# ska-sa/dc_sand

Measured on AMD Instinct MI355X. Metric: Gcoeff/s (complex weights) 64ant x 1024beam x 32768chan per GPU, higher is better.
Workload: dtype f32

## Files before the change

### dc_sand_amd/csrc/bf_capi_stream.hip

```cpp

#include <cstring>
#include <new>

#include "../../include/dcs_stream_staging.h"
#include "bf_stream_ext.h"
#include "bf_host.h"

using namespace bf_host;

constexpr int kTableRing = 4;
struct dcs_bf_stream {
    bf_stream_ext_head ext;
    dcs_bf_context *ctx;
    hipStream_t stream;
    hipGraph_t graph;
    hipGraphExec_t exec;
    hipGraphNode_t node;
    bf_kernel_launch launch;
    bool has_terms;
    hipGraphNode_t terms_node;
    bf_terms_args terms_args;
    const void *terms_func;
    dim3 terms_grid, terms_block;
    dcs_delay_vals *h_table[kTableRing];
    hipEvent_t table_copied[kTableRing];
    bool table_pending[kTableRing];
    int table_next;
    hipGraph_t ggraph;
    hipGraphExec_t gexec;
    hipGraphNode_t gnode_gather, gnode_terms, gnode_gen;
    bf_gather_launch gather;
    dcs_delay_vals *d_spare;
    hipStream_t stage_stream;
    hipEvent_t staged_ev;
    hipEvent_t released_ev;
    bool released_recorded;
    bool staged;
};

namespace {

void kernel_node_params(const bf_kernel_launch &l, void **params, hipKernelNodeParams *np)
{
    std::memset(np, 0, sizeof(*np));
    np->func = const_cast<void *>(l.func);
    np->gridDim = l.grid;
    np->blockDim = l.block;
    np->sharedMemBytes = l.shared;
    np->kernelParams = params;
    np->extra = nullptr;
}

void terms_node_params(const dcs_bf_stream *s, void **params, hipKernelNodeParams *tp)
{
    std::memset(tp, 0, sizeof(*tp));
    tp->func = const_cast<void *>(s->terms_func);
    tp->gridDim = s->terms_grid;
    tp->blockDim = s->terms_block;
    tp->kernelParams = params;
}

void gather_node_params(dcs_bf_stream *s, void **params, hipKernelNodeParams *gp)
{
    bf_gather_launch &g = s->gather;
    params[0] = &g.local;
    params[1] = &g.global;
    params[2] = &g.n_ant;
    params[3] = &g.nb_local;
    params[4] = &g.nb_total;
    params[5] = &g.beam_offset;
    std::memset(gp, 0, sizeof(*gp));
    gp->func = const_cast<void *>(g.func);
    gp->gridDim = g.grid;
    gp->blockDim = g.block;
    gp->kernelParams = params;
}

int build_stream_graph(dcs_bf_stream *s, bool with_gather, hipGraph_t *graph, hipGraphExec_t *exec, hipGraphNode_t *n_gather,
                       hipGraphNode_t *n_terms, hipGraphNode_t *n_gen)
{
    DCS_TRY(hipGraphCreate(graph, 0));
    hipGraphNode_t prev = nullptr;
    if (with_gather) {
        void *gparams[6];
        hipKernelNodeParams gp;
        gather_node_params(s, gparams, &gp);
        DCS_TRY(hipGraphAddKernelNode(n_gather, *graph, nullptr, 0, &gp));
        prev = *n_gather;
    }
    if (s->has_terms) {
        void *tparams[] = {&s->terms_args};
        hipKernelNodeParams tp;
        terms_node_params(s, tparams, &tp);
        DCS_TRY(hipGraphAddKernelNode(n_terms, *graph, prev ? &prev : nullptr, prev ? 1 : 0, &tp));
        prev = *n_terms;
    }
    void *params[] = {&s->launch.args};
    hipKernelNodeParams np;
    kernel_node_params(s->launch, params, &np);
    DCS_TRY(hipGraphAddKernelNode(n_gen, *graph, prev ? &prev : nullptr, prev ? 1 : 0, &np));
    DCS_TRY(hipGraphInstantiate(exec, *graph, nullptr, nullptr, 0));
    return DCS_OK;
}

int replay(dcs_bf_stream *s, float dt, const dcs_delay_vals *delays, hipGraphExec_t exec, hipGraphNode_t n_gather,
           hipGraphNode_t n_terms, hipGraphNode_t n_gen)
{
    s->launch.args.a.dt0 = dt;
    s->launch.args.a.delays = delays;
    if (n_gather) {
        void *gparams[6];
        hipKernelNodeParams gp;
        gather_node_params(s, gparams, &gp);
        DCS_TRY(hipGraphExecKernelNodeSetParams(exec, n_gather, &gp));
    }
    if (s->has_terms) {
        s->terms_args.dt0 = dt;
        s->terms_args.dt_inline[0] = dt;
        s->terms_args.delays = delays;
        void *tparams[] = {&s->terms_args};
        hipKernelNodeParams tp;
        terms_node_params(s, tparams, &tp);
        DCS_TRY(hipGraphExecKernelNodeSetParams(exec, n_terms, &tp));
    }
    void *params[] = {&s->launch.args};
    hipKernelNodeParams np;
    kernel_node_params(s->launch, params, &np);
    DCS_TRY(hipGraphExecKernelNodeSetParams(exec, n_gen, &np));
    return (int)hipGraphLaunch(exec, s->stream);
}

int ensure_staging(dcs_bf_stream *s)
{
    if (!s->d_spare) DCS_TRY(hipMalloc((void **)&s->d_spare, (size_t)s->ctx->n_pairs * sizeof(dcs_delay_vals)));
    if (!s->stage_stream) {
        int least = 0, greatest = 0;
        DCS_TRY(hipDeviceGetStreamPriorityRange(&least, &greatest));
        DCS_TRY(hipStreamCreateWithPriority(&s->stage_stream, hipStreamNonBlocking, greatest));
    }
    if (!s->staged_ev) DCS_TRY(hipEventCreateWithFlags(&s->staged_ev, hipEventDisableTiming));
    if (!s->released_ev) DCS_TRY(hipEventCreateWithFlags(&s->released_ev, hipEventDisableTiming));
    return DCS_OK;
}

int begin_staging(dcs_bf_stream *s)
{
    const int cap = refuse_if_capturing(s->stream);
    if (cap != DCS_OK) return cap;
    const int st = ensure_staging(s);
    if (st != DCS_OK) return st;
    if (s->released_recorded) DCS_TRY(hipStreamWaitEvent(s->stage_stream, s->released_ev, 0));
    return DCS_OK;
}

int consume_staged(dcs_bf_stream *s, float dt)
{
    dcs_bf_context *c = s->ctx;
    DCS_TRY(hipStreamWaitEvent(s->stream, s->staged_ev, 0));
    DCS_TRY(hipEventRecord(s->released_ev, s->stream));
    s->released_recorded = true;
    const int st = replay(s, dt, s->d_spare, s->exec, nullptr, s->terms_node, s->node);
    if (st != DCS_OK) return st;
    dcs_delay_vals *retired = c->d_table[c->cur];
    c->d_table[c->cur] = s->d_spare;
    s->d_spare = retired;
    s->staged = false;
    return DCS_OK;
}

int stage_table_impl(dcs_bf_stream *s, const dcs_delay_vals *table, int flags)
{
    if (!s || !table) return DCS_ERR_INVALID_ARGUMENT;
    if (flags != 0 && flags != DCS_BF_STAGE_CALLER_PINNED) return DCS_ERR_INVALID_ARGUMENT;
    dcs_bf_context *c = s->ctx;
    DCS_CHECK_DEVICE(c);
    const size_t tb = (size_t)c->n_pairs * sizeof(dcs_delay_vals);
    const int st = begin_staging(s);
    if (st != DCS_OK) return st;
    const void *src = table;
    int r = -1;
    if (flags == 0) {
        r = s->table_next;
        s->table_next = (r + 1) % kTableRing;
        if (s->table_pending[r]) DCS_TRY(hipEventSynchronize(s->table_copied[r]));
        std::memcpy(s->h_table[r], table, tb);
        src = s->h_table[r];
    }
    DCS_TRY(hipMemcpyAsync(s->d_spare, src, tb, hipMemcpyHostToDevice, s->stage_stream));
    if (r >= 0) {
        DCS_TRY(hipEventRecord(s->table_copied[r], s->stage_stream));
        s->table_pending[r] = true;
    }
    DCS_TRY(hipEventRecord(s->staged_ev, s->stage_stream));
    s->staged = true;
    return DCS_OK;
}

int stage_table_from_global_impl(dcs_bf_stream *s, const void *d_global, uint32_t nb_total, uint32_t beam_offset,
                                 void *ready_event)
{
    if (!s || !d_global) return DCS_ERR_INVALID_ARGUMENT;
    dcs_bf_context *c = s->ctx;
    DCS_CHECK_DEVICE(c);
    if ((uint64_t)beam_offset + (uint64_t)c->p.nr_beams > nb_total) return DCS_ERR_OUT_OF_RANGE;
    if ((reinterpret_cast<uintptr_t>(d_global) & 15u) != 0) return DCS_ERR_INVALID_ARGUMENT;
    const int st = begin_staging(s);
    if (st != DCS_OK) return st;
    if (ready_event) DCS_TRY(hipStreamWaitEvent(s->stage_stream, reinterpret_cast<hipEvent_t>(ready_event), 0));
    DCS_TRY(bf_launch_gather_beams(s->d_spare, static_cast<const dcs_delay_vals *>(d_global), (uint32_t)c->p.nr_stations,
                                   (uint32_t)c->p.nr_beams, nb_total, beam_offset, s->stage_stream));
    DCS_TRY(hipEventRecord(s->staged_ev, s->stage_stream));
    s->staged = true;
    return DCS_OK;
}

const bf_stream_ext_ops kStagingOps = {BF_STREAM_EXT_VERSION, stage_table_impl, stage_table_from_global_impl};

}

extern "C" {

int dcs_bf_stream_begin(dcs_bf_context *c, int bitwidth, uint32_t c0, uint32_t nc, void *d_out, size_t out_bytes,
                        void *stream, dcs_bf_stream **out)
{
    if (!c || !out || !d_out) return DCS_ERR_INVALID_ARGUMENT;
    DCS_CHECK_DEVICE(c);
    *out = nullptr;
    if (bitwidth != DCS_BF_B16 && bitwidth != DCS_BF_B32) return DCS_ERR_INVALID_ARGUMENT;
    if (!c->table_set) return DCS_ERR_NOT_READY;
    if ((uint64_t)c0 + nc > (uint64_t)c->p.nr_channels || nc == 0) return DCS_ERR_OUT_OF_RANGE;
    const bool out16 = bitwidth == DCS_BF_B16;
    if (out_bytes < (size_t)nc * c->n_pairs * (out16 ? 4 : 8)) return DCS_ERR_INVALID_ARGUMENT;
    {
        const int cap = refuse_if_capturing(as_stream(stream));
        if (cap != DCS_OK) return cap;
    }

    dcs_bf_stream *s = new (std::nothrow) dcs_bf_stream();
    if (!s) return (int)hipErrorOutOfMemory;
    std::memset(static_cast<void *>(s), 0, sizeof(*s));
    s->ext.ops = &kStagingOps;
    s->ctx = c;
    s->stream = as_stream(stream);
    int st = DCS_OK;
    do {
        s->has_terms = want_terms_table(c, out16, pick_geometry(c, out16, nc, 1), nc, 1);
        if ((st = prepare_tiled(c, out16, nullptr, 0.0f, 1, c0, nc, d_out, &s->launch, nullptr, s->has_terms)) != 0) break;
        if (s->launch.func == nullptr) { st = DCS_ERR_INVALID_ARGUMENT; break; }
        if (s->has_terms) {
            fill_terms_table_args(c, out16, 0.0f, 1, c0, nc, d_out, nullptr, &s->terms_args);
            if ((st = (int)bf_prepare_terms(s->terms_args, &s->terms_func, &s->terms_grid, &s->terms_block)) != 0) break;
            if (s->terms_func == nullptr) { st = DCS_ERR_INVALID_ARGUMENT; break; }
        }
        if ((st = (int)bf_prepare_gather_beams(c->d_table[c->cur ^ 1], c->d_table[c->cur], (uint32_t)c->p.nr_stations,
                                               (uint32_t)c->p.nr_beams, (uint32_t)c->p.nr_beams, 0u, &s->gather)) != 0) break;
        if (s->gather.func == nullptr) { st = DCS_ERR_INVALID_ARGUMENT; break; }
        for (int i = 0; i < kTableRing && st == 0; i++) {
            st = (int)hipHostMalloc((void **)&s->h_table[i], (size_t)c->n_pairs * sizeof(dcs_delay_vals), hipHostMallocDefault);
            if (st == 0) st = (int)hipEventCreateWithFlags(&s->table_copied[i], hipEventDisableTiming);
        }
        if (st != 0) break;
        if ((st = build_stream_graph(s, false, &s->graph, &s->exec, nullptr, &s->terms_node, &s->node)) != 0) break;
        if ((st = build_stream_graph(s, true, &s->ggraph, &s->gexec, &s->gnode_gather, &s->gnode_terms, &s->gnode_gen)) != 0) break;
    } while (0);
    if (st != 0) {
        dcs_bf_stream_end(s);
        return st;
    }
    *out = s;
    return DCS_OK;
}

int dcs_bf_stream_tick_dt(dcs_bf_stream *s, float dt, const dcs_delay_vals *new_table)
{
    if (!s) return DCS_ERR_INVALID_ARGUMENT;
    dcs_bf_context *c = s->ctx;
    DCS_CHECK_DEVICE(c);
    if (s->staged) return new_table ? DCS_ERR_INVALID_ARGUMENT : consume_staged(s, dt);
    if (new_table) {
        const int r = s->table_next;
        s->table_next = (r + 1) % kTableRing;
        if (s->table_pending[r]) DCS_TRY(hipEventSynchronize(s->table_copied[r]));
        std::memcpy(s->h_table[r], new_table, (size_t)c->n_pairs * sizeof(dcs_delay_vals));
        const int nxt = c->cur ^ 1;
        DCS_TRY(hipMemcpyAsync(c->d_table[nxt], s->h_table[r], (size_t)c->n_pairs * sizeof(dcs_delay_vals),
                               hipMemcpyHostToDevice, s->stream));
        DCS_TRY(hipEventRecord(s->table_copied[r], s->stream));
        s->table_pending[r] = true;
        c->cur = nxt;
    }
    return replay(s, dt, c->d_table[c->cur], s->exec, nullptr, s->terms_node, s->node);
}

int dcs_bf_stream_tick(dcs_bf_stream *s, uint64_t t, const dcs_delay_vals *new_table)
{
    if (!s) return DCS_ERR_INVALID_ARGUMENT;
    float dt;
    const int st = dcs_bf_delta_times(&s->ctx->p, t, 1, &dt);
    if (st != DCS_OK) return st;
    return dcs_bf_stream_tick_dt(s, dt, new_table);
}

int dcs_bf_stream_tick_at(dcs_bf_stream *s, const struct timespec *cur, const struct timespec *ref,
                          const dcs_delay_vals *new_table)
{
    if (!s) return DCS_ERR_INVALID_ARGUMENT;
    float dt;
    const int st = dcs_bf_ts_diff(ref, cur, &dt);
    if (st != DCS_OK) return st;
    return dcs_bf_stream_tick_dt(s, dt, new_table);
}

int dcs_bf_stream_tick_dt_from_global(dcs_bf_stream *s, float dt, const void *d_global, uint32_t nb_total, uint32_t beam_offset)
{
    if (!s || !d_global) return DCS_ERR_INVALID_ARGUMENT;
    dcs_bf_context *c = s->ctx;
    DCS_CHECK_DEVICE(c);
    if ((uint64_t)beam_offset + (uint64_t)c->p.nr_beams > nb_total) return DCS_ERR_OUT_OF_RANGE;
    if ((reinterpret_cast<uintptr_t>(d_global) & 15u) != 0) return DCS_ERR_INVALID_ARGUMENT;
    if (s->staged) return DCS_ERR_INVALID_ARGUMENT;
    const int nxt = c->cur ^ 1;
    s->gather.local = c->d_table[nxt];
    s->gather.global = static_cast<const dcs_delay_vals *>(d_global);
    s->gather.nb_total = nb_total;
    s->gather.beam_offset = beam_offset;
    c->cur = nxt;
    return replay(s, dt, c->d_table[c->cur], s->gexec, s->gnode_gather, s->gnode_terms, s->gnode_gen);
}

int dcs_bf_stream_tick_from_global(dcs_bf_stream *s, uint64_t t, const void *d_global, uint32_t nb_total, uint32_t beam_offset)
{
    if (!s) return DCS_ERR_INVALID_ARGUMENT;
    float dt;
    const int st = dcs_bf_delta_times(&s->ctx->p, t, 1, &dt);
    if (st != DCS_OK) return st;
    return dcs_bf_stream_tick_dt_from_global(s, dt, d_global, nb_total, beam_offset);
}

int dcs_bf_stream_tick_at_from_global(dcs_bf_stream *s, const struct timespec *cur, const struct timespec *ref,
                                      const void *d_global, uint32_t nb_total, uint32_t beam_offset)
{
    if (!s) return DCS_ERR_INVALID_ARGUMENT;
    float dt;
    const int st = dcs_bf_ts_diff(ref, cur, &dt);
    if (st != DCS_OK) return st;
    return dcs_bf_stream_tick_dt_from_global(s, dt, d_global, nb_total, beam_offset);
}

int dcs_bf_stream_end(dcs_bf_stream *s)
{
    if (!s) return DCS_OK;
    (void)hipStreamSynchronize(s->stream);
    if (s->stage_stream) {
        (void)hipStreamSynchronize(s->stage_stream);
        (void)hipStreamDestroy(s->stage_stream);
    }
    if (s->staged_ev) (void)hipEventDestroy(s->staged_ev);
    if (s->released_ev) (void)hipEventDestroy(s->released_ev);
    if (s->d_spare) (void)hipFree(s->d_spare);
    if (s->exec) (void)hipGraphExecDestroy(s->exec);
    if (s->graph) (void)hipGraphDestroy(s->graph);
    if (s->gexec) (void)hipGraphExecDestroy(s->gexec);
    if (s->ggraph) (void)hipGraphDestroy(s->ggraph);
    for (int i = 0; i < kTableRing; i++) {
        if (s->table_copied[i]) (void)hipEventDestroy(s->table_copied[i]);
        if (s->h_table[i]) (void)hipHostFree(s->h_table[i]);
    }
    delete s;
    return DCS_OK;
}

}
```

### include/dcs_probes.h

```cpp
#ifndef DCS_PROBES_H
#define DCS_PROBES_H

#include "dcs_beamformer.h"

#ifdef __cplusplus
extern "C" {
#endif
#pragma GCC visibility push(default)

struct dcs_probe_knobs {
    int32_t nomath;
    int32_t pace;
    int32_t fail_at_step;
    int32_t bacc_probe;
    int32_t bacc_rounds;
    int32_t bacc_no_share;
    int32_t bacc_plain;
    int32_t bacc_wg_per_cu;
    int32_t bacc_unstaged;
    int32_t bacc_order;
    int32_t bacc_nbt;
    int32_t bacc_waves;
};
int dcs_probe_set_knobs(dcs_bf_context *ctx, const struct dcs_probe_knobs *k);

int dcs_probe_sincos(int which, const float *d_x, size_t n, float *d_sin, float *d_cos, void *stream);
int dcs_probe_fill(void *d_out, size_t bytes, int nontemporal, void *stream);
int dcs_probe_store_pattern(void *d_out, uint32_t rows, uint32_t cols_kib, uint32_t qb, uint32_t rb, int order,
                            int xcd_remap, int nontemporal, uint32_t block_threads, void *stream);

int dcs_probe_one_store(void *d_out, size_t bytes, int store_mode, int stores_per_thread, uint32_t row_bytes, void *stream);

int dcs_probe_reduce(const void *d_in, size_t bytes, uint64_t *checksum, float *max_modulus_dev, void *stream);

int dcs_probe_mfma(int which, uint32_t blocks, uint32_t iters, float *d_out, void *stream);

uint32_t dcs_probe_xcd_grouped(uint32_t w, uint32_t total, uint32_t group);

int dcs_probe_copy(const void *d_in, void *d_out, size_t bytes, int store_mode, int per_thread, void *stream);

#pragma GCC visibility pop
#ifdef __cplusplus
}
#endif
#endif
```

### probes/dcs_probes.py

```python
from __future__ import annotations

import ctypes
from ctypes import POINTER, byref, c_float, c_int, c_size_t, c_uint32, c_uint64, c_void_p

import numpy as np

from .build import LIB, build

_VP = c_void_p
SIGNATURES = [
    ("dcs_probe_sincos", c_int, [c_int, _VP, c_size_t, _VP, _VP, _VP]),
    ("dcs_probe_fill", c_int, [_VP, c_size_t, c_int, _VP]),
    ("dcs_probe_copy", c_int, [_VP, _VP, c_size_t, c_int, c_int, _VP]),
    ("dcs_probe_one_store", c_int, [_VP, c_size_t, c_int, c_int, c_uint32, _VP]),
    ("dcs_probe_reduce", c_int, [_VP, c_size_t, POINTER(c_uint64), POINTER(c_float), _VP]),
    ("dcs_probe_mfma", c_int, [c_int, c_uint32, c_uint32, _VP, _VP]),
    ("dcs_probe_store_pattern", c_int, [_VP, c_uint32, c_uint32, c_uint32, c_uint32, c_int, c_int, c_int, c_uint32, _VP]),
    ("dcs_probe_set_knobs", c_int, [_VP, _VP]),
    ("dcs_probe_xcd_grouped", c_uint32, [c_uint32, c_uint32, c_uint32]),
]

KNOB_FIELDS = ("nomath", "pace", "fail_at_step", "bacc_probe", "bacc_rounds", "bacc_no_share", "bacc_plain", "bacc_wg_per_cu",
               "bacc_unstaged", "bacc_order", "bacc_nbt", "bacc_waves")

_LIB = None


def lib() -> ctypes.CDLL:
    global _LIB
    if _LIB is None:
        if not LIB.exists():
            build()
        L = ctypes.CDLL(str(LIB))
        for name, restype, argtypes in SIGNATURES:
            fn = getattr(L, name)
            fn.restype = restype
            fn.argtypes = argtypes
        _LIB = L
    return _LIB


def _check(status: int, where: str) -> None:
    if status != 0:
        raise RuntimeError(f"{where}: status {status}")


def _s(stream) -> c_void_p:
    if stream is None:
        return c_void_p(None)
    return c_void_p(int(getattr(stream, "handle", stream)))


def tensor_properties(d_ptr, nbytes: int, stream=None) -> tuple[int, float]:
    ck = c_uint64(0)
    dev = c_float(0.0)
    _check(lib().dcs_probe_reduce(c_void_p(int(d_ptr)), int(nbytes), byref(ck), byref(dev), _s(stream)), "dcs_probe_reduce")
    return int(ck.value), float(dev.value)


def sincos(which: int, d_x, n: int, d_sin, d_cos, stream=None) -> None:
    _check(lib().dcs_probe_sincos(int(which), c_void_p(int(d_x)), int(n), c_void_p(int(d_sin)), c_void_p(int(d_cos)), _s(stream)),
           "dcs_probe_sincos")


def fill(d_out, nbytes: int, nontemporal: int = 1, stream=None) -> None:
    _check(lib().dcs_probe_fill(c_void_p(int(d_out)), int(nbytes), int(nontemporal), _s(stream)), "dcs_probe_fill")


def copy(d_in, d_out, nbytes: int, store_mode: int = 1, per_thread: int = 1, stream=None) -> None:
    _check(lib().dcs_probe_copy(c_void_p(int(d_in)), c_void_p(int(d_out)), int(nbytes), int(store_mode), int(per_thread), _s(stream)),
           "dcs_probe_copy")


def store_pattern(d_out, rows, cols_kib, qb, rb, order=0, xcd_remap=0, store_mode=1, block_threads=256, stream=None) -> None:
    _check(lib().dcs_probe_store_pattern(c_void_p(int(d_out)), rows, cols_kib, qb, rb, order, xcd_remap, store_mode, block_threads,
                                         _s(stream)), "dcs_probe_store_pattern")


def one_store(d_out, nbytes, store_mode, stores_per_thread, row_bytes, stream=None) -> None:
    _check(lib().dcs_probe_one_store(c_void_p(int(d_out)), int(nbytes), int(store_mode), int(stores_per_thread), int(row_bytes),
                                     _s(stream)), "dcs_probe_one_store")


def mfma(which: int, blocks: int, iters: int, d_out, stream=None) -> None:
    _check(lib().dcs_probe_mfma(int(which), int(blocks), int(iters), c_void_p(int(d_out)), _s(stream)), "dcs_probe_mfma")


def set_knobs(gen, **knobs) -> None:
    from dc_sand_amd import _lib as product

    if product.LIB_PATH.resolve() != LIB.resolve():
        raise RuntimeError("set_knobs needs the probes build behind the wrappers: run with DCS_LIB_PATH=probes/libdcs_probes.so")
    unknown = set(knobs) - set(KNOB_FIELDS)
    if unknown:
        raise TypeError(f"unknown knob(s) {sorted(unknown)}")
    if not knobs:
        _check(lib().dcs_probe_set_knobs(c_void_p(gen._h), c_void_p(None)), "dcs_probe_set_knobs")
        return
    k = (ctypes.c_int32 * len(KNOB_FIELDS))(*[int(knobs.get(f, 0)) for f in KNOB_FIELDS])
    _check(lib().dcs_probe_set_knobs(c_void_p(gen._h), ctypes.cast(k, c_void_p)), "dcs_probe_set_knobs")
```

Before: 927.9.

## Route host-table ticks through the staging stream and add stream-join probe knob

When a tick carries a new host delay table, the upload now goes on the high-priority staging stream and joins the compute stream through events, instead of being copied inline on the compute stream. The aim is to let the H2D copy overlap the previous generation kernel rather than serialize ahead of it. A probe knob adds variants that drop the wait, drop or move the release event, or disable the system fence, for measuring the join cost. This adds event record and wait calls per tick, and the no-wait and no-release probe variants give up ordering guarantees.

```diff
diff --git a/dc_sand_amd/csrc/bf_capi_stream.hip b/dc_sand_amd/csrc/bf_capi_stream.hip
--- a/dc_sand_amd/csrc/bf_capi_stream.hip
+++ b/dc_sand_amd/csrc/bf_capi_stream.hip
@@ -130,6 +130,8 @@
     return (int)hipGraphLaunch(exec, s->stream);
 }
 
+constexpr int kJoinNoRelease = 1, kJoinNoWait = 2, kJoinNoSystemFence = 3, kJoinRecordBehind = 4;
+
 int ensure_staging(dcs_bf_stream *s)
 {
     if (!s->d_spare) DCS_TRY(hipMalloc((void **)&s->d_spare, (size_t)s->ctx->n_pairs * sizeof(dcs_delay_vals)));
@@ -139,7 +141,11 @@
         DCS_TRY(hipStreamCreateWithPriority(&s->stage_stream, hipStreamNonBlocking, greatest));
     }
     if (!s->staged_ev) DCS_TRY(hipEventCreateWithFlags(&s->staged_ev, hipEventDisableTiming));
-    if (!s->released_ev) DCS_TRY(hipEventCreateWithFlags(&s->released_ev, hipEventDisableTiming));
+    if (!s->released_ev) {
+        unsigned flags = hipEventDisableTiming;
+        if (DCS_PROBE_KNOB(s->ctx, stream_join) == kJoinNoSystemFence) flags |= hipEventDisableSystemFence;
+        DCS_TRY(hipEventCreateWithFlags(&s->released_ev, flags));
+    }
     return DCS_OK;
 }
 
@@ -153,45 +159,82 @@
     return DCS_OK;
 }
 
-int consume_staged(dcs_bf_stream *s, float dt)
-{
-    dcs_bf_context *c = s->ctx;
-    DCS_TRY(hipStreamWaitEvent(s->stream, s->staged_ev, 0));
-    DCS_TRY(hipEventRecord(s->released_ev, s->stream));
-    s->released_recorded = true;
-    const int st = replay(s, dt, s->d_spare, s->exec, nullptr, s->terms_node, s->node);
-    if (st != DCS_OK) return st;
-    dcs_delay_vals *retired = c->d_table[c->cur];
-    c->d_table[c->cur] = s->d_spare;
-    s->d_spare = retired;
-    s->staged = false;
-    return DCS_OK;
-}
-
-int stage_table_impl(dcs_bf_stream *s, const dcs_delay_vals *table, int flags)
-{
-    if (!s || !table) return DCS_ERR_INVALID_ARGUMENT;
-    if (flags != 0 && flags != DCS_BF_STAGE_CALLER_PINNED) return DCS_ERR_INVALID_ARGUMENT;
-    dcs_bf_context *c = s->ctx;
-    DCS_CHECK_DEVICE(c);
-    const size_t tb = (size_t)c->n_pairs * sizeof(dcs_delay_vals);
-    const int st = begin_staging(s);
-    if (st != DCS_OK) return st;
+int copy_host_table(dcs_bf_stream *s, const dcs_delay_vals *table, bool caller_pinned, dcs_delay_vals *dst, hipStream_t stream)
+{
+    const size_t tb = (size_t)s->ctx->n_pairs * sizeof(dcs_delay_vals);
     const void *src = table;
     int r = -1;
-    if (flags == 0) {
+    if (!caller_pinned) {
         r = s->table_next;
         s->table_next = (r + 1) % kTableRing;
         if (s->table_pending[r]) DCS_TRY(hipEventSynchronize(s->table_copied[r]));
         std::memcpy(s->h_table[r], table, tb);
         src = s->h_table[r];
     }
-    DCS_TRY(hipMemcpyAsync(s->d_spare, src, tb, hipMemcpyHostToDevice, s->stage_stream));
+    DCS_TRY(hipMemcpyAsync(dst, src, tb, hipMemcpyHostToDevice, stream));
     if (r >= 0) {
-        DCS_TRY(hipEventRecord(s->table_copied[r], s->stage_stream));
+        DCS_TRY(hipEventRecord(s->table_copied[r], stream));
         s->table_pending[r] = true;
     }
+    return DCS_OK;
+}
+
+int stage_host_table(dcs_bf_stream *s, const dcs_delay_vals *table, bool caller_pinned)
+{
+    const int st = copy_host_table(s, table, caller_pinned, s->d_spare, s->stage_stream);
+    if (st != DCS_OK) return st;
     DCS_TRY(hipEventRecord(s->staged_ev, s->stage_stream));
+    return DCS_OK;
+}
+
+int consume_staged(dcs_bf_stream *s, float dt)
+{
+    dcs_bf_context *c = s->ctx;
+    const int join = DCS_PROBE_KNOB(c, stream_join);
+    if (join != kJoinNoWait) DCS_TRY(hipStreamWaitEvent(s->stream, s->staged_ev, 0));
+    if (join != kJoinNoRelease && join != kJoinRecordBehind) {
+        DCS_TRY(hipEventRecord(s->released_ev, s->stream));
+        s->released_recorded = true;
+    }
+    const int st = replay(s, dt, s->d_spare, s->exec, nullptr, s->terms_node, s->node);
+    if (st != DCS_OK) return st;
+    if (join == kJoinRecordBehind) DCS_TRY(hipEventRecord(s->released_ev, s->stream));
+    dcs_delay_vals *retired = c->d_table[c->cur];
+    c->d_table[c->cur] = s->d_spare;
+    s->d_spare = retired;
+    s->staged = false;
+    return DCS_OK;
+}
+
+int tick_with_host_table(dcs_bf_stream *s, float dt, const dcs_delay_vals *table)
+{
+    dcs_bf_context *c = s->ctx;
+    hipStreamCaptureStatus cs = hipStreamCaptureStatusNone;
+    bool overlapped = hipStreamIsCapturing(s->stream, &cs) == hipSuccess && cs == hipStreamCaptureStatusNone;
+    if (overlapped && ensure_staging(s) != DCS_OK) {
+        (void)hipGetLastError();
+        overlapped = false;
+    }
+    if (overlapped) {
+        if (s->released_recorded) DCS_TRY(hipStreamWaitEvent(s->stage_stream, s->released_ev, 0));
+        const int st = stage_host_table(s, table, false);
+        return st != DCS_OK ? st : consume_staged(s, dt);
+    }
+    const int nxt = c->cur ^ 1;
+    const int st = copy_host_table(s, table, false, c->d_table[nxt], s->stream);
+    if (st != DCS_OK) return st;
+    c->cur = nxt;
+    return replay(s, dt, c->d_table[c->cur], s->exec, nullptr, s->terms_node, s->node);
+}
+
+int stage_table_impl(dcs_bf_stream *s, const dcs_delay_vals *table, int flags)
+{
+    if (!s || !table) return DCS_ERR_INVALID_ARGUMENT;
+    if (flags != 0 && flags != DCS_BF_STAGE_CALLER_PINNED) return DCS_ERR_INVALID_ARGUMENT;
+    DCS_CHECK_DEVICE(s->ctx);
+    int st = begin_staging(s);
+    if (st == DCS_OK) st = stage_host_table(s, table, flags == DCS_BF_STAGE_CALLER_PINNED);
+    if (st != DCS_OK) return st;
     s->staged = true;
     return DCS_OK;
 }
@@ -277,18 +320,7 @@
     dcs_bf_context *c = s->ctx;
     DCS_CHECK_DEVICE(c);
     if (s->staged) return new_table ? DCS_ERR_INVALID_ARGUMENT : consume_staged(s, dt);
-    if (new_table) {
-        const int r = s->table_next;
-        s->table_next = (r + 1) % kTableRing;
-        if (s->table_pending[r]) DCS_TRY(hipEventSynchronize(s->table_copied[r]));
-        std::memcpy(s->h_table[r], new_table, (size_t)c->n_pairs * sizeof(dcs_delay_vals));
-        const int nxt = c->cur ^ 1;
-        DCS_TRY(hipMemcpyAsync(c->d_table[nxt], s->h_table[r], (size_t)c->n_pairs * sizeof(dcs_delay_vals),
-                               hipMemcpyHostToDevice, s->stream));
-        DCS_TRY(hipEventRecord(s->table_copied[r], s->stream));
-        s->table_pending[r] = true;
-        c->cur = nxt;
-    }
+    if (new_table) return tick_with_host_table(s, dt, new_table);
     return replay(s, dt, c->d_table[c->cur], s->exec, nullptr, s->terms_node, s->node);
 }
 
diff --git a/include/dcs_probes.h b/include/dcs_probes.h
--- a/include/dcs_probes.h
+++ b/include/dcs_probes.h
@@ -21,6 +21,7 @@
     int32_t bacc_order;
     int32_t bacc_nbt;
     int32_t bacc_waves;
+    int32_t stream_join;
 };
 int dcs_probe_set_knobs(dcs_bf_context *ctx, const struct dcs_probe_knobs *k);
 
diff --git a/probes/dcs_probes.py b/probes/dcs_probes.py
--- a/probes/dcs_probes.py
+++ b/probes/dcs_probes.py
@@ -21,7 +21,7 @@
 ]
 
 KNOB_FIELDS = ("nomath", "pace", "fail_at_step", "bacc_probe", "bacc_rounds", "bacc_no_share", "bacc_plain", "bacc_wg_per_cu",
-               "bacc_unstaged", "bacc_order", "bacc_nbt", "bacc_waves")
+               "bacc_unstaged", "bacc_order", "bacc_nbt", "bacc_waves", "stream_join")
 
 _LIB = None
 
```

Measured after the change: 928.2, median of 2. No clear change (+0.0%).
